# meteorologytoday/XLab-FFTBarotropic

Measured on AMD Instinct MI355X. Metric: RK4 steps/sec, 4096x4096 periodic grid, higher is better.
Workload: dtype f32; 1 GPU; 4096x4096 kuo2004 initial field, nu=6.5, L=600 km, dt=0.75 s, 4 RK stages/step, fused HIP path; parallelism=single

## Files before the change

### __graft_entry__.py

```python
import os
import sys
import time

ROOT = os.path.dirname(os.path.abspath(__file__))
for p in (ROOT, os.path.join(ROOT, "oracle")):
    if p not in sys.path:
        sys.path.insert(0, p)


def csrc_digest():
    import hashlib
    h = hashlib.sha256()
    d = os.path.join(ROOT, "xlab-fftbarotropic_amd", "csrc")
    for f in sorted(os.listdir(d)) + [os.path.join(ROOT, "tools", "build_variant.sh"), os.path.join(ROOT, "include", "fftbaro.h")]:
        h.update(open(f if os.path.isabs(f) else os.path.join(d, f), "rb").read())
    return h.hexdigest()


def build():
    import xlab_fftbarotropic_amd as X
    X.build_lib(force=not os.path.exists(X.package.build.LIB))
    L = X.lib()
    missing = [n for n in X.EXPORTS if not hasattr(L, n)]
    if missing:
        raise RuntimeError("libfftbaro.so lacks %s" % missing)
    import subprocess
    subprocess.check_call(["make", "-s", "-C", os.path.join(ROOT, "xlab-fftbarotropic_amd", "host")])
    import oracle_py
    oracle_py.build()
    oracle_py.lib()
    alt = os.path.join(ROOT, "xlab-fftbarotropic_amd", "lib", "alt_nozc_prebuilt.so")
    digest = csrc_digest()
    stamp = alt + ".sha"
    if not (os.path.exists(alt) and os.path.exists(stamp) and open(stamp).read().strip() == digest):
        if os.path.exists(stamp):
            os.remove(stamp)
        t0 = time.time()
        subprocess.check_call([os.path.join(ROOT, "tools", "build_variant.sh"), "nozc_prebuilt", "-DCF_REMAKE_ZC=0", "-DFB_MID_REMAKE_ZC=0"],
                              stdout=subprocess.DEVNULL)
        if not os.path.exists(alt) or os.path.getmtime(alt) < t0 - 1.0:
            raise RuntimeError("tools/build_variant.sh returned 0 but %s was not rebuilt" % alt)
        if csrc_digest() != digest:
            raise RuntimeError("the engine's sources changed while the variant library was being built")
        open(stamp, "w").write(digest + "\n")
    return None


def smoke():
    import numpy as np
    import torch
    import xlab_fftbarotropic_amd as X
    import oracle_py as O
    assert torch.cuda.is_available(), "smoke() needs a GPU"
    torch.cuda.set_device(0)
    n = 256
    v0 = O.make_field("elliptic", n)
    m = X.Model(n, n)
    m.set_vort(v0)
    m.step(5)
    got = m.vort().cpu().numpy()
    mo = O.Model(n, n)
    mo.set_vort(v0)
    mo.step(5)
    want = mo.vort()
    err = float(np.linalg.norm((got - want).astype(np.float64)) / np.linalg.norm(want.astype(np.float64)))
    assert err < 1e-5, "smoke parity failed: rel L2 = %g" % err
    print("smoke ok: 256^2 elliptic vortex, 5 RK4 steps, rel L2 vs oracle = %.3g" % err)
    return None


if __name__ == "__main__":
    build()
    if len(sys.argv) > 1 and sys.argv[1] == "smoke":
        smoke()
```

### xlab-fftbarotropic_amd/csrc/fb_col_full.h

```cpp
#pragma once
#include "fb_kernels.h"

#define CF_THREADS 1024
#define CF_X1_CF 16384
#define CF_X2_STR 68
#define CF_X2_CF (16 * 16 * CF_X2_STR)
#define CF_GX_CF 2048
#define CF_LDS_CF (CF_X2_CF + 512 + CF_GX_CF)
#define CF_LDS_BYTES (CF_LDS_CF * 8)

struct FullArgs {
    const cf *Tin;
    const cf *Zbase;
    cf *Zcur, *Acc, *Zout;
    cf *W4;
    long fstride;
    int P;
    int ntiles;
    int ntiles_run;
    int nsub;
    int stage;
    float nu, dt;
    SpecCoef coef;
    const cf *tw256;
    const cf *tw4096;
    long sub_rows;
    float wscale;
};

FB_DEV void cf_xchg_waves(cf *lds, cf *v, int w, int lane)
{
#pragma unroll
    for (int r = 0; r < 16; ++r) lds_wr(&lds[(r * 16 + w) * 64 + lane], v[r]);
    lds_barrier();
#pragma unroll
    for (int r = 0; r < 16; ++r) v[r] = lds_rd(&lds[(w * 16 + r) * 64 + lane]);
    lds_barrier();
}

template <bool SYNC>
FB_DEV void cf_xchg_lanes(cf *lds, cf *v, int w, int l, int c)
{
    cf *reg = lds + w * (16 * CF_X2_STR);
#pragma unroll
    for (int r = 0; r < 16; ++r) lds_wr(&reg[r * CF_X2_STR + l * 4 + c], v[r]);
    __builtin_amdgcn_wave_barrier();
#pragma unroll
    for (int r = 0; r < 16; ++r) v[r] = lds_rd(&reg[l * CF_X2_STR + r * 4 + c]);
    if (SYNC) lds_barrier();
    else { asm volatile("s_waitcnt lgkmcnt(0)" ::: "memory"); __builtin_amdgcn_wave_barrier(); }
}

#define CF_FENCE() __builtin_amdgcn_sched_barrier(0)
FB_DEV cf cf_mul(cf a, cf b) { return cmul_split(a, b); }
FB_DEV cf cf_mulc(cf a, cf b) { return cmulc_split(a, b); }

template <int DIR> FB_DEV void cf_bfly16(cf *v)
{
    fft4<DIR>(v[0], v[4], v[8], v[12]);  CF_FENCE();
    fft4<DIR>(v[1], v[5], v[9], v[13]);  CF_FENCE();
    fft4<DIR>(v[2], v[6], v[10], v[14]); CF_FENCE();
    fft4<DIR>(v[3], v[7], v[11], v[15]); CF_FENCE();
    v[5]  = mul_w16<1, DIR, true>(v[5]);  v[6]  = mul_w16<2, DIR, true>(v[6]);  v[7]  = mul_w16<3, DIR, true>(v[7]);
    v[9]  = mul_w16<2, DIR, true>(v[9]);  v[10] = mul_w16<4, DIR, true>(v[10]); v[11] = mul_w16<6, DIR, true>(v[11]);
    v[13] = mul_w16<3, DIR, true>(v[13]); v[14] = mul_w16<6, DIR, true>(v[14]); v[15] = mul_w16<9, DIR, true>(v[15]);
    CF_FENCE();
    fft4<DIR>(v[0], v[1], v[2], v[3]);     CF_FENCE();
    fft4<DIR>(v[4], v[5], v[6], v[7]);     CF_FENCE();
    fft4<DIR>(v[8], v[9], v[10], v[11]);   CF_FENCE();
    fft4<DIR>(v[12], v[13], v[14], v[15]); CF_FENCE();
    cf t;
    t = v[1];  v[1]  = v[4];  v[4]  = t;
    t = v[2];  v[2]  = v[8];  v[8]  = t;
    t = v[3];  v[3]  = v[12]; v[12] = t;
    t = v[6];  v[6]  = v[9];  v[9]  = t;
    t = v[7];  v[7]  = v[13]; v[13] = t;
    t = v[11]; v[11] = v[14]; v[14] = t;
}

template <int DIR>
FB_DEV void cf_fft4096(cf *lds, const cf *tabA, const cf *tabB, cf (*v)[16], int w, int l, int c, int lane)
{
    if (DIR < 0) {
#pragma unroll
        for (int col = 0; col < 2; ++col) {
            cf_bfly16<-1>(v[col]);
#pragma unroll
            for (int k1 = 1; k1 < 16; ++k1) { v[col][k1] = cf_mul(v[col][k1], tabB[w * k1]); if ((k1 & 3) == 3) CF_FENCE(); }
            cf_xchg_waves(lds, v[col], w, lane);
            CF_FENCE();
        }
        const cf a = tabA[l * w];
#pragma unroll
        for (int col = 0; col < 2; ++col) {
            cf_bfly16<-1>(v[col]);
            v[col][0] = cf_mul(v[col][0], a);
#pragma unroll
            for (int k2 = 1; k2 < 16; ++k2) { v[col][k2] = cf_mul(v[col][k2], cf_mul(a, tabB[l * k2])); if ((k2 & 3) == 3) CF_FENCE(); }
            cf_xchg_lanes<false>(lds, v[col], w, l, c);
            CF_FENCE();
        }
#pragma unroll
        for (int col = 0; col < 2; ++col) { cf_bfly16<-1>(v[col]); CF_FENCE(); }
    } else {
#pragma unroll
        for (int col = 0; col < 2; ++col) {
            cf_bfly16<+1>(v[col]);
#pragma unroll
            for (int lr = 1; lr < 16; ++lr) { v[col][lr] = cf_mulc(v[col][lr], cf_mul(tabA[lr * w], tabB[lr * l])); if ((lr & 3) == 3) CF_FENCE(); }
            if (col == 0) cf_xchg_lanes<false>(lds, v[col], w, l, c);
            else cf_xchg_lanes<true>(lds, v[col], w, l, c);
            CF_FENCE();
        }
#pragma unroll
        for (int col = 0; col < 2; ++col) {
            cf_bfly16<+1>(v[col]);
#pragma unroll
            for (int wr = 1; wr < 16; ++wr) { v[col][wr] = cf_mulc(v[col][wr], tabB[wr * w]); if ((wr & 3) == 3) CF_FENCE(); }
            cf_xchg_waves(lds, v[col], w, lane);
            CF_FENCE();
        }
#pragma unroll
        for (int col = 0; col < 2; ++col) { cf_bfly16<+1>(v[col]); CF_FENCE(); }
    }
}

FB_DEV float4 cf_ld4(const void *ubase, unsigned voff) { return *reinterpret_cast<const float4 *>(static_cast<const char *>(ubase) + voff); }
FB_DEV void cf_st4(void *ubase, unsigned voff, float4 x) { *reinterpret_cast<float4 *>(static_cast<char *>(ubase) + voff) = x; }
FB_DEV void cf_st4_w4(void *ubase, unsigned voff, float4 x) { st4<true>(static_cast<char *>(ubase) + voff, x); }

template <int STAGE, int NSUB>
__global__ void __launch_bounds__(CF_THREADS) k_col_full(FullArgs a)
{
    extern __shared__ __attribute__((aligned(16))) unsigned char smem_raw[];
    cf *lds = reinterpret_cast<cf *>(smem_raw);
    cf *tabB = lds + CF_X2_CF, *tabA = tabB + 256;
    float *gxt = reinterpret_cast<float *>(tabA + 256);
    const int tid = threadIdx.x, lane = tid & 63, l = lane >> 2, c = lane & 3;
    const int w = __builtin_amdgcn_readfirstlane(tid >> 6);

    constexpr int nsub = NSUB;
    const int ntg = gridDim.x / nsub;
    const int k1 = NSUB == 1 ? 0 : blockIdx.x / ntg, bt = blockIdx.x - k1 * ntg;
    int tile = bt;
    if ((ntg & 7) == 0) tile = (bt & 7) * (ntg >> 3) + (bt >> 3);
    if (tile >= a.ntiles_run) return;

    const int ky0 = tile * 8 + 2 * c;
    const unsigned voff_m = (unsigned)((l * a.P + 2 * c) * (int)sizeof(cf));
    const size_t ubase_m = ((size_t)(k1 * a.sub_rows + 16 * w) * a.P + (size_t)tile * 8) * sizeof(cf);
    const size_t rstep = (size_t)256 * a.P * sizeof(cf);
    const unsigned voff_s = (unsigned)(lane * (int)sizeof(float4));
    const size_t ubase_s = ((((size_t)k1 * (a.ntiles + 1) + tile) * 16) * CF_THREADS + (size_t)w * 64) * sizeof(float4);
    const size_t sstep = (size_t)CF_THREADS * sizeof(float4);

    constexpr bool PRIME = STAGE == 4;
    cf v[2][16];
    {
        const char *src = reinterpret_cast<const char *>(a.Tin) + ubase_m;
        float4 tin[16];
        if (!PRIME) {
#pragma unroll
            for (int i = 0; i < 16; ++i) tin[i] = ld4<true>(src + i * rstep + voff_m);
        }
        float g4[4];
#pragma unroll
        for (int i = 0; i < 4; ++i) g4[i] = a.coef.gx[nsub * (tid + i * CF_THREADS) + k1];
        if (tid < 256) { tabB[tid] = a.tw256[tid]; tabA[tid] = a.tw4096[tid]; }
#pragma unroll
        for (int i = 0; i < 4; ++i) {
            const int ik = tid + i * CF_THREADS;
            gxt[((ik >> 4) & 15) + 16 * (ik & 15) + (ik & ~255)] = g4[i];
        }
        if (!PRIME) {
#pragma unroll
            for (int i = 0; i < 16; ++i) { v[0][i] = cf_make(tin[i].x, tin[i].y); v[1][i] = cf_make(tin[i].z, tin[i].w); }
        }
    }
    __syncthreads();
    if (!PRIME) cf_fft4096<-1>(lds, tabA, tabB, v, w, l, c, lane);

    const char *Z0 = reinterpret_cast<const char *>(a.Zbase) + ubase_s;
    char *ZC = reinterpret_cast<char *>(a.Zcur) + ubase_s, *AC = reinterpret_cast<char *>(a.Acc) + ubase_s,
         *ZO = reinterpret_cast<char *>(a.Zout) + ubase_s;
    const float gya = a.coef.gy[ky0], gyb = a.coef.gy[ky0 + 1];
    auto ky2_of = [](float g) { asm volatile("" : "+v"(g)); return (double)g * (double)g; };
    constexpr bool PRIME_ = STAGE == 4;
    const bool pada = PRIME_ && ky0 >= a.coef.hy, padb = PRIME_ && ky0 + 1 >= a.coef.hy;
    constexpr int stage = STAGE;
    const float nu = a.nu, dt = a.dt, hdt = (stage == 2) ? a.dt : a.dt / 2.0f;
    constexpr int DEPTH = STAGE == 0 ? 2 : 1;
#ifndef CF_REMAKE_ZC
#define CF_REMAKE_ZC 1
#endif
    constexpr bool REMAKE_ZC = CF_REMAKE_ZC && STAGE == 1;
    float4 q0[DEPTH], q1[DEPTH], q2[DEPTH];
    auto load_k3 = [&](int k3) {
        const int sl = k3 % DEPTH;
        q0[sl] = ld4<false>(Z0 + k3 * sstep + voff_s);
        if (stage != 0) q2[sl] = ld4<true>(AC + k3 * sstep + voff_s);
        if (stage != 0 && !REMAKE_ZC) q1[sl] = ld4<false>(ZC + k3 * sstep + voff_s);
    };
    if (!PRIME) {
#pragma unroll
        for (int k3 = 0; k3 < DEPTH; ++k3) load_k3(k3);
    }
#pragma unroll
    for (int k3 = 0; k3 < (PRIME ? 0 : 16); ++k3) {
        const int sl = k3 % DEPTH;
        const int ik2 = w + 256 * k3 + 16 * l, ikx = nsub * ik2 + k1;
        const float gx = gxt[l + 16 * w + 256 * k3];
        const double kx2 = (double)gx * (double)gx;
        const float lapa = (float)(-(kx2 + ky2_of(gya))), lapb = (float)(-(kx2 + ky2_of(gyb)));
        const float mska = coef_mask(a.coef, ikx, ky0), mskb = coef_mask(a.coef, ikx, ky0 + 1);
        const float4 z0 = q0[sl];
        float4 zc = z0;
        if (REMAKE_ZC) {
            const float4 ac = q2[sl];
            zc = make_float4(__builtin_fmaf(ac.x, hdt, z0.x), __builtin_fmaf(ac.y, hdt, z0.y), __builtin_fmaf(ac.z, hdt, z0.z), __builtin_fmaf(ac.w, hdt, z0.w));
        } else if (stage != 0) zc = q1[sl];
        float4 k;
        k.x = (v[0][k3].x + (zc.x * lapa) * nu) * mska; k.y = (v[0][k3].y + (zc.y * lapa) * nu) * mska;
        k.z = (v[1][k3].x + (zc.z * lapb) * nu) * mskb; k.w = (v[1][k3].y + (zc.w * lapb) * nu) * mskb;
        float4 acc, zn;
        if (stage == 0) {
            acc = k;
            zn = make_float4(__builtin_fmaf(k.x, hdt, z0.x), __builtin_fmaf(k.y, hdt, z0.y), __builtin_fmaf(k.z, hdt, z0.z), __builtin_fmaf(k.w, hdt, z0.w));
        } else if (stage < 3) {
            const float4 ac = q2[sl];
            acc = make_float4(ac.x + 2.0f * k.x, ac.y + 2.0f * k.y, ac.z + 2.0f * k.z, ac.w + 2.0f * k.w);
            zn = make_float4(z0.x + k.x * hdt, z0.y + k.y * hdt, z0.z + k.z * hdt, z0.w + k.w * hdt);
        } else {
            const float4 ac = q2[sl];
            acc = ac;
            zn = make_float4(z0.x + (ac.x + k.x) * dt / 6.0f, z0.y + (ac.y + k.y) * dt / 6.0f,
                             z0.z + (ac.z + k.z) * dt / 6.0f, z0.w + (ac.w + k.w) * dt / 6.0f);
        }
        v[0][k3] = cf_make(zn.x, zn.y); v[1][k3] = cf_make(zn.z, zn.w);
        if (k3 + DEPTH < 16) load_k3(k3 + DEPTH);
        if (stage < 3) { st4<true>(AC + k3 * sstep + voff_s, acc); cf_st4(ZC + k3 * sstep, voff_s, zn); }
        else cf_st4(ZO + k3 * sstep, voff_s, zn);
        CF_FENCE();
    }

    const char *ZN = PRIME ? Z0 : (stage < 3 ? ZC : ZO);
#pragma unroll 1
    for (int f = 0; f < 4; ++f) {
        if (f > 0 || PRIME) {
            const unsigned vs = (unsigned)launder((int)voff_s);
#pragma unroll
            for (int k3 = 0; k3 < 16; ++k3) {
                const float4 z = cf_ld4(ZN + k3 * sstep, vs);
                v[0][k3] = cf_make(z.x, z.y); v[1][k3] = cf_make(z.z, z.w);
            }
        }
        const bool psi = f >= 2, use_gx = (f == 0 || f == 3);
        const int lkx = launder(l);
#pragma unroll
        for (int k3 = 0; k3 < 16; ++k3) {
            cf za = v[0][k3], zb = v[1][k3];
            const float gx = gxt[16 * w + 256 * k3 + lkx];
            if (psi) {
                const double kx2 = (double)gx * (double)gx;
                const float lia = (nsub * (w + 256 * k3 + 16 * l) + k1 == 0 && ky0 == 0) ? 1.0f : (float)(-(kx2 + ky2_of(gya)));
                const float lib = (float)(-(kx2 + ky2_of(gyb)));
                za = pada ? cf_make(0.f, 0.f) : cf_make(za.x / lia, za.y / lia);
                zb = padb ? cf_make(0.f, 0.f) : cf_make(zb.x / lib, zb.y / lib);
            }
            const float ka = (use_gx ? gx : gya) * a.wscale, kb = (use_gx ? gx : gyb) * a.wscale;
            v[0][k3] = cf_make(-za.y * ka, za.x * ka);
            v[1][k3] = cf_make(-zb.y * kb, zb.x * kb);
            CF_FENCE();
        }
        cf_fft4096<+1>(lds, tabA, tabB, v, w, l, c, lane);
        char *dst = reinterpret_cast<char *>(a.W4) + (size_t)f * a.fstride * sizeof(cf) + ubase_m;
        const unsigned vm = (unsigned)launder((int)voff_m);
#pragma unroll
        for (int i = 0; i < 16; ++i)
            cf_st4_w4(dst + i * rstep, vm, make_float4(v[0][i].x, v[0][i].y, v[1][i].x, v[1][i].y));
    }
}

template <bool TO_FULL>
__global__ void __launch_bounds__(256) k_full_relayout(const cf *__restrict__ in, cf *__restrict__ out, int P, int N1, int N2, int ntiles, int nsub, int hy)
{
    const size_t total = (size_t)nsub * (ntiles + 1) * 16 * CF_THREADS * 2;
    for (size_t idx = (size_t)blockIdx.x * blockDim.x + threadIdx.x; idx < total; idx += (size_t)gridDim.x * blockDim.x) {
        const int col = (int)(idx & 1);
        const int tid = (int)((idx >> 1) & (CF_THREADS - 1));
        const int k3 = (int)((idx >> 11) & 15);
        const int st = (int)(idx >> 15);
        const int k1 = st / (ntiles + 1), tile = st - k1 * (ntiles + 1);
        const int w = tid >> 6, l = (tid >> 2) & 15, c = tid & 3;
        const int kx = nsub * (w + 16 * l + 256 * k3) + k1, ky = tile * 8 + 2 * c + col;
        const int cc = kx % N1, d = kx / N1;
        const size_t p3 = (size_t)(N2 * cc + d) * P + ky;
        if (ky >= hy) { if (TO_FULL) out[idx] = cf_make(0.f, 0.f); continue; }
        if (TO_FULL) out[idx] = in[p3]; else out[p3] = in[idx];
    }
}
```

Before: 1220 steps/s.

## Skip global loads/stores for fully masked spectral blocks via buffer-rsrc zero-size trick

Computes a per-wave bitmask of k3 blocks whose spectral dealias mask is zero at both corners, then issues loads and stores through AMD buffer resources with num_records set to zero for those blocks. Out-of-range buffer accesses become no-ops, so masked blocks skip Acc/Zcur traffic, and the next FFT pass reads Zbase instead. This targets memory bandwidth spent on truncated wavenumbers, at the cost of extra mask evaluation, buffer-instruction overhead, and reliance on the block-corner test being valid for the mask shape. A no-skip variant library is also built in parallel for comparison.

```diff
diff --git a/__graft_entry__.py b/__graft_entry__.py
--- a/__graft_entry__.py
+++ b/__graft_entry__.py
@@ -29,15 +29,21 @@
     import oracle_py
     oracle_py.build()
     oracle_py.lib()
-    alt = os.path.join(ROOT, "xlab-fftbarotropic_amd", "lib", "alt_nozc_prebuilt.so")
+    variants = (("nozc_prebuilt", ["-DCF_REMAKE_ZC=0", "-DFB_MID_REMAKE_ZC=0"]), ("noblockskip_prebuilt", ["-DCF_NO_BLOCK_SKIP"]))
     digest = csrc_digest()
-    stamp = alt + ".sha"
-    if not (os.path.exists(alt) and os.path.exists(stamp) and open(stamp).read().strip() == digest):
+    jobs = []
+    for name, flags in variants:
+        alt = os.path.join(ROOT, "xlab-fftbarotropic_amd", "lib", "alt_%s.so" % name)
+        stamp = alt + ".sha"
+        if os.path.exists(alt) and os.path.exists(stamp) and open(stamp).read().strip() == digest:
+            continue
         if os.path.exists(stamp):
             os.remove(stamp)
-        t0 = time.time()
-        subprocess.check_call([os.path.join(ROOT, "tools", "build_variant.sh"), "nozc_prebuilt", "-DCF_REMAKE_ZC=0", "-DFB_MID_REMAKE_ZC=0"],
-                              stdout=subprocess.DEVNULL)
+        jobs.append((alt, stamp, time.time(), subprocess.Popen([os.path.join(ROOT, "tools", "build_variant.sh"), name] + flags, stdout=subprocess.DEVNULL)))
+    failed = [alt for alt, _, _, p in jobs if p.wait() != 0]
+    if failed:
+        raise RuntimeError("tools/build_variant.sh failed for %s" % failed)
+    for alt, stamp, t0, _ in jobs:
         if not os.path.exists(alt) or os.path.getmtime(alt) < t0 - 1.0:
             raise RuntimeError("tools/build_variant.sh returned 0 but %s was not rebuilt" % alt)
         if csrc_digest() != digest:
diff --git a/xlab-fftbarotropic_amd/csrc/fb_col_full.h b/xlab-fftbarotropic_amd/csrc/fb_col_full.h
--- a/xlab-fftbarotropic_amd/csrc/fb_col_full.h
+++ b/xlab-fftbarotropic_amd/csrc/fb_col_full.h
@@ -129,6 +129,36 @@
 FB_DEV void cf_st4(void *ubase, unsigned voff, float4 x) { *reinterpret_cast<float4 *>(static_cast<char *>(ubase) + voff) = x; }
 FB_DEV void cf_st4_w4(void *ubase, unsigned voff, float4 x) { st4<true>(static_cast<char *>(ubase) + voff, x); }
 
+FB_DEV unsigned cf_block_mask(const SpecCoef &c, int nsub, int k1, int w, int tile)
+{
+    unsigned m = 0;
+#pragma unroll
+    for (int k3 = 0; k3 < 16; ++k3) {
+        const int kx0 = nsub * (w + 256 * k3) + k1, kx15 = kx0 + nsub * 240;
+        if (coef_mask(c, kx0, tile * 8) == 0.0f && coef_mask(c, kx15, tile * 8) == 0.0f) m |= 1u << k3;
+    }
+    return (unsigned)__builtin_amdgcn_readfirstlane((int)m);
+}
+
+typedef unsigned cf_u4v __attribute__((ext_vector_type(4)));
+typedef float cf_f4v __attribute__((ext_vector_type(4)));
+#define CF_BLK_BYTES (64 * 16)
+#define CF_BUF_NT 2
+FB_DEV __amdgpu_buffer_rsrc_t cf_blk_rsrc(const void *blk, bool frozen)
+{
+    return __builtin_amdgcn_make_buffer_rsrc(const_cast<void *>(blk), 0, frozen ? 0 : CF_BLK_BYTES, 0x00020000);
+}
+template <bool NT> FB_DEV float4 cf_blk_ld4(const void *blk, bool frozen, unsigned voff)
+{
+    const cf_f4v r = __builtin_bit_cast(cf_f4v, __builtin_amdgcn_raw_buffer_load_b128(cf_blk_rsrc(blk, frozen), (int)voff, 0, NT ? CF_BUF_NT : 0));
+    return make_float4(r[0], r[1], r[2], r[3]);
+}
+template <bool NT> FB_DEV void cf_blk_st4(void *blk, bool frozen, unsigned voff, float4 x)
+{
+    const cf_f4v r = {x.x, x.y, x.z, x.w};
+    __builtin_amdgcn_raw_buffer_store_b128(__builtin_bit_cast(cf_u4v, r), cf_blk_rsrc(blk, frozen), (int)voff, 0, NT ? CF_BUF_NT : 0);
+}
+
 template <int STAGE, int NSUB>
 __global__ void __launch_bounds__(CF_THREADS) k_col_full(FullArgs a)
 {
@@ -194,9 +224,23 @@
 #define CF_REMAKE_ZC 1
 #endif
     constexpr bool REMAKE_ZC = CF_REMAKE_ZC && STAGE == 1;
+#ifdef CF_NO_BLOCK_SKIP
+    constexpr bool BSKIP = false;
+#else
+    constexpr bool BSKIP = !PRIME;
+#endif
+    const unsigned bmask = BSKIP ? cf_block_mask(a.coef, nsub, k1, w, tile) : 0u;
+    auto frozen = [&](int k3) { return BSKIP && ((bmask >> k3) & 1u) != 0; };
+    const bool zo_inplace = a.Zout == a.Zbase;
     float4 q0[DEPTH], q1[DEPTH], q2[DEPTH];
     auto load_k3 = [&](int k3) {
         const int sl = k3 % DEPTH;
+        if (BSKIP) {
+            q0[sl] = cf_blk_ld4<false>(Z0 + k3 * sstep, false, voff_s);
+            if (stage != 0) q2[sl] = cf_blk_ld4<true>(AC + k3 * sstep, frozen(k3), voff_s);
+            if (stage != 0 && !REMAKE_ZC) q1[sl] = cf_blk_ld4<false>(ZC + k3 * sstep, frozen(k3), voff_s);
+            return;
+        }
         q0[sl] = ld4<false>(Z0 + k3 * sstep + voff_s);
         if (stage != 0) q2[sl] = ld4<true>(AC + k3 * sstep + voff_s);
         if (stage != 0 && !REMAKE_ZC) q1[sl] = ld4<false>(ZC + k3 * sstep + voff_s);
@@ -236,9 +280,13 @@
             zn = make_float4(z0.x + (ac.x + k.x) * dt / 6.0f, z0.y + (ac.y + k.y) * dt / 6.0f,
                              z0.z + (ac.z + k.z) * dt / 6.0f, z0.w + (ac.w + k.w) * dt / 6.0f);
         }
+        if (frozen(k3)) zn = z0;
         v[0][k3] = cf_make(zn.x, zn.y); v[1][k3] = cf_make(zn.z, zn.w);
         if (k3 + DEPTH < 16) load_k3(k3 + DEPTH);
-        if (stage < 3) { st4<true>(AC + k3 * sstep + voff_s, acc); cf_st4(ZC + k3 * sstep, voff_s, zn); }
+        if (BSKIP) {
+            if (stage < 3) { cf_blk_st4<true>(AC + k3 * sstep, frozen(k3), voff_s, acc); cf_blk_st4<false>(ZC + k3 * sstep, frozen(k3), voff_s, zn); }
+            else cf_blk_st4<false>(ZO + k3 * sstep, frozen(k3) && zo_inplace, voff_s, zn);
+        } else if (stage < 3) { st4<true>(AC + k3 * sstep + voff_s, acc); cf_st4(ZC + k3 * sstep, voff_s, zn); }
         else cf_st4(ZO + k3 * sstep, voff_s, zn);
         CF_FENCE();
     }
@@ -250,7 +298,8 @@
             const unsigned vs = (unsigned)launder((int)voff_s);
 #pragma unroll
             for (int k3 = 0; k3 < 16; ++k3) {
-                const float4 z = cf_ld4(ZN + k3 * sstep, vs);
+                const char *zsrc = (frozen(k3) ? Z0 : ZN) + k3 * sstep;
+                const float4 z = BSKIP ? cf_blk_ld4<false>(zsrc, false, vs) : cf_ld4(zsrc, vs);
                 v[0][k3] = cf_make(z.x, z.y); v[1][k3] = cf_make(z.z, z.w);
             }
         }
```

New measurement: 1220 steps/s. No clear change (-0.0%).
